# sclipman/gfa2network

Hardware: AMD Instinct MI355X
Metric: M edges/sec GFA->CSR (device-resident), + GB/s ingested (higher is better)
Workload: dtype u8/int64 (float64 weights); 1 GPU; C4: 50M S / 200M L, default (directed, MAX-SYM CSR), HBM-resident parse; n_segments=50000000, n_links=200000000, input_bytes_per_gpu=6299989066, n_nodes=50000000, nnz=289480899, mode=default, output=csr, parallelism=replica x1

## Files before the change

gfa2network_amd/_native.py:

```python
from __future__ import annotations

import ctypes
import os
import sys
from dataclasses import dataclass, field
from pathlib import Path

import numpy as np

LIB_PATH = Path(__file__).resolve().parent / "_lib" / "libg2n.so"

ABI_VERSION = 2
MAX_PHASES = 40

OK = 0
E_MALFORMED_L, E_MALFORMED_E, E_MALFORMED_C, E_MALFORMED_P, E_MALFORMED_O = 1, 2, 3, 4, 5
E_INDEX_LIST, E_INDEX_BYTES, E_UNICODE, E_INT_TOO_LARGE = 6, 7, 8, 9
E_CAST_OVERFLOW, E_CAST_INF, E_CAST_NAN = 10, 11, 12
E_ARG, E_IO, E_GZIP, E_DEVICE, E_NOMEM, E_UNSUPPORTED = 13, 14, 15, 16, 17, 18

DTYPE_CODES = {"bool": 0, "int8": 1, "int32": 2, "float32": 3, "float64": 4}
CODE_DTYPES = {v: np.dtype(k) for k, v in DTYPE_CODES.items()}
OUT_PARSE, OUT_CSR, OUT_COO, OUT_EDGE_LIST = 0, 1, 2, 3
FMT_COO, FMT_CSR, FMT_TEXT = 0, 1, 2

EXPORTED = [
    "g2n_version", "g2n_abi_version", "g2n_options_init", "g2n_device_count", "g2n_device_memory", "g2n_last_error",
    "g2n_status_name", "g2n_release_shared", "g2n_build_from_path", "g2n_build_from_buffer", "g2n_result_free",
    "g2n_coo_to_csr", "g2n_coo_to_csr_band", "g2n_context_create", "g2n_context_destroy", "g2n_context_stream", "g2n_context_trim",
    "g2n_build_device", "g2n_build_decimal_range", "g2n_count_device", "g2n_order_keys", "g2n_rank_keys", "g2n_upload_file_range", "g2n_partition_keys", "g2n_dedup_keys", "g2n_gather_keys", "g2n_remap_pairs", "g2n_route_triplets", "g2n_csr_from_coo_pair",
    "g2n_context_group_slots", "g2n_route_group_slots", "g2n_csr_from_group_slots",
    "g2n_keyset_create", "g2n_keyset_add", "g2n_keyset_view", "g2n_keyset_free",
    "g2n_gunzip", "g2n_gunzip_chunked", "g2n_free", "g2n_split_render", "g2n_split_get", "g2n_split_segments", "g2n_split_free", "g2n_join_names", "g2n_gather_names", "g2n_write_npz", "g2n_write_node_map", "g2n_first_bad_utf8",
    "g2n_csr_stats", "g2n_csr_stats_host", "g2n_stats_from_path",
]


TEST_NO_BUCKETS = 2
TEST_NO_LEAN = 4
TEST_DICT_HASH = 8
TEST_DICT_GENERAL = 16
TEST_NO_TILE_LOCAL = 32
TEST_HOST_INFLATE = 64
TEST_NO_GROUP = 128
TEST_NO_HASH_LEAN = 256
TEST_THROW_AFTER_IDS = 512
TEST_INDEX64 = 1024
TEST_DICT_DIRECT = 2048
TEST_NO_DIRECT = 4096
TEST_NO_EXT_LEAN = 8192
TEST_NO_DEC_TEXT = 16384
TEST_NO_DEC_PREFIX = 32768
TEST_FLAGS = int(os.environ.get("G2N_TEST_FLAGS", "0"), 0)
RANGE_DECIMAL = 1
RANGE_EVIDENCE = 2
RANGE_NO_VALUES = 4
RANGE_SLOTS = 8


class Options(ctypes.Structure):
    _fields_ = [
        ("abi_version", ctypes.c_uint32),
        ("directed", ctypes.c_int32),
        ("bidirected", ctypes.c_int32),
        ("keep_directed_bidir", ctypes.c_int32),
        ("asymmetric", ctypes.c_int32),
        ("strip_orientation", ctypes.c_int32),
        ("dtype", ctypes.c_int32),
        ("output", ctypes.c_int32),
        ("weight_tag", ctypes.c_char_p),
        ("want_node_names", ctypes.c_int32),
        ("device", ctypes.c_int32),
        ("unknown_warned", ctypes.c_int32),
        ("range_flags", ctypes.c_int32),
        ("range_s_base", ctypes.c_int64),
        ("range_n_segments", ctypes.c_int64),
        ("test_flags", ctypes.c_uint32),
        ("reserved_", ctypes.c_int32 * 3),
    ]


class Result(ctypes.Structure):
    _fields_ = [
        ("abi_version", ctypes.c_uint32),
        ("status", ctypes.c_int32),
# ... 697 lines not shown
```

gfa2network_amd/csrc/g2n_pipeline.hip:

```cpp
#include <hip/hip_runtime.h>

#include <chrono>
#include <cstring>
#include <functional>
#include <map>
#include <memory>
#include <mutex>

#include "g2n_internal.h"
#include "g2n_kernels.hip"
#include "g2n_scan.hip"
#include "g2n_sort.hip"
#include "g2n_sym.hip"
#include "g2n_route.hip"
#include "g2n_inflate.hip"
#include "g2n_keyset.hip"
#include "g2n_stats.hip"

#define G2N_HIP(call)                                                                                      \
  do {                                                                                                     \
    hipError_t e_ = (call);                                                                                \
    if (e_ != hipSuccess)                                                                                  \
      throw ::g2n::Failure(G2N_E_DEVICE, std::string(#call " failed: ") + hipGetErrorString(e_));          \
  } while (0)

namespace g2n {

enum Slot {
  S_IN, S_TILE_CNT, S_TILE_BASE, S_LS, S_KIND, S_NOFF, S_NLEN, S_OOFF, S_OLEN, S_EW, S_ETB, S_WL, S_TABLE,
  S_SLOT, S_FIRST, S_NID, S_FLEN, S_BLOB, S_OFFS, S_ROWS, S_COLS, S_DATA, S_KEYS0, S_KEYS1, S_VALS0, S_VALS1,
  S_KV, S_ODATA, S_INDPTR, S_INDICES, S_TEMP, S_WT, S_TKIND, S_TSTATE, S_RSTART0, S_RSTART1, S_ROUT0,
  S_ROUT1, S_UCNT0, S_UCNT1, S_UOFF, S_MCNT, S_MOFF, S_RSCR, S_RFLAG0, S_RFLAG1, S_RVAL0, S_RVAL1, S_TID,
  S_INV, S_TUNK, S_DEFER, S_FOFF64, S_BTC, S_BTV, S_BTOT, S_EBAD, S_ELEN, S_EPOS, S_ETEXT, S_EFIRST, S_EMETA, S_EL0, S_EL1,
  S_PCNT, S_POFF, S_PGRP, S_BSTART, S_SCANST, S_RBOUND, S_ROWSP, S_COLSP, S_TLEAN, S_ZIN, S_ZMEM, S_ZBAD, S_RSK, S_RSV, S_RSCNT, S_RSOFF,
  S_GCNT, S_TCN, S_INDPTR64, S_INDICES64, S_WENC, S_W1, S_W2, S_TVAL, S_PW0, S_PW1, S_BSTARTA, S_DIRECT, S_RTOT, S_SCANST2, S_EWP, S_TLIST, S_TNB, S_WENCP,
  S_STPARENT, S_STCOL, S_STDIAG, S_STLONG, S_STOUT, S_STIP, S_STIX,
  S_NSLOTS
};

constexpr uint64_t kMinGroups = 1024;
constexpr uint32_t kPtileSmallDiv = 4;
constexpr uint32_t kF2Ranges = 4;
constexpr uint32_t kTestNoBuckets = G2N_TEST_NO_BUCKETS;
constexpr uint32_t kTestNoLean = G2N_TEST_NO_LEAN;
constexpr uint32_t kTestDictHash = G2N_TEST_DICT_HASH;
constexpr uint32_t kTestDictGeneral = G2N_TEST_DICT_GENERAL;
constexpr uint32_t kTestNoTileLocal = G2N_TEST_NO_TILE_LOCAL;
constexpr uint32_t kTestNoGroup = G2N_TEST_NO_GROUP;
constexpr uint32_t kTestNoHashLean = G2N_TEST_NO_HASH_LEAN;
constexpr uint32_t kTestThrowAfterIds = G2N_TEST_THROW_AFTER_IDS;
constexpr uint32_t kTestIndex64 = G2N_TEST_INDEX64;
constexpr uint32_t kTestDictDirect = G2N_TEST_DICT_DIRECT;
constexpr uint32_t kTestNoDirect = G2N_TEST_NO_DIRECT;
constexpr uint32_t kTestNoExtLean = G2N_TEST_NO_EXT_LEAN;
constexpr uint32_t kTestNoDecText = G2N_TEST_NO_DEC_TEXT;
constexpr uint32_t kTestNoDecPrefix = G2N_TEST_NO_DEC_PREFIX;


struct DevBuf {
  void* p = nullptr;
  size_t cap = 0;
  uint64_t call = 0;
};
struct ScanSlot {
  void* p = nullptr;
  size_t cap = 0;
  uint32_t epoch = 0;
  uint64_t ticket = 0;
};

struct GroupedCoo {
  bool active = false;
  bool failed = false;
  const int32_t* rows = nullptr;
  const int32_t* cols = nullptr;
  const uint32_t* gcount = nullptr;
  uint64_t gcap = 0, n_groups = 0;
  const uint32_t* wenc = nullptr;
};

}

struct g2n_context {
  int device = 0;
  int n_cu = 256;
  uint32_t test_flags = 0;
  uint64_t err_line_off = 0;
  g2n::GroupedCoo gcoo;
  g2n::GroupedCoo slots;
// ... 334 lines not shown
  const bool words = !t_rows && (sum || !pair);
  const uint32_t ptile = n_el >= (1ull << 24) ? kPartTile : kPartTile / kPtileSmallDiv;
  src.tile = ptile;
  const uint64_t n_blk1 = grouped ? c->gcoo.n_groups : (n_el + ptile - 1) / ptile;
  const uint64_t nm1 = (uint64_t)n_dig1 * n_blk1;
  auto* cnt1 = dget<uint32_t>(c, S_PCNT, (words ? 2 : 1) * nm1);
  auto* off1 = dget<uint32_t>(c, S_POFF, (words ? 2 : 1) * nm1);
  auto* el1 = dget<uint2>(c, S_EL0, n_el);
  uint32_t* wa1 = words ? dget<uint32_t>(c, S_PW0, n_trip) : nullptr;
  if (sum && !t_rows) {
    src.pair_bits = (uint32_t)low + 1u;
    hipLaunchKernelGGL(k_part_hist<4>, dim3((unsigned)n_blk1), dim3(kPartTPB), 0, c->stream, src, shift1, n_dig1,
                       cnt1, n_blk1);
    scan_excl<uint32_t, uint32_t>(c, cnt1, off1, 2 * nm1);
    hipLaunchKernelGGL(k_part_scatter<4>, dim3((unsigned)n_blk1), dim3(kPartTPB), 0, c->stream, src, shift1, n_dig1,
                       (const uint32_t*)off1, n_blk1, el1, wa1);
  } else if (sum || pair) {
    hipLaunchKernelGGL(k_part_hist<3>, dim3((unsigned)n_blk1), dim3(kPartTPB), 0, c->stream, src, shift1, n_dig1,
                       cnt1, n_blk1);
    scan_excl<uint32_t, uint32_t>(c, cnt1, off1, (uint64_t)n_dig1 * n_blk1);
    hipLaunchKernelGGL(k_part_scatter<3>, dim3((unsigned)n_blk1), dim3(kPartTPB), 0, c->stream, src, shift1, n_dig1,
                       (const uint32_t*)off1, n_blk1, el1);
  } else {
    hipLaunchKernelGGL(k_part_hist<1>, dim3((unsigned)n_blk1), dim3(kPartTPB), 0, c->stream, src, shift1, n_dig1,
                       cnt1, n_blk1);
    scan_excl<uint32_t, uint32_t>(c, cnt1, off1, 2 * nm1);
    hipLaunchKernelGGL(k_part_scatter<1>, dim3((unsigned)n_blk1), dim3(kPartTPB), 0, c->stream, src, shift1, n_dig1,
                       (const uint32_t*)off1, n_blk1, el1, wa1);
  }
  auto* bst = dget<uint32_t>(c, S_BSTART, n_buckets + 1);
  uint32_t* bstA = words ? dget<uint32_t>(c, S_BSTARTA, n_buckets + 1) : nullptr;
  const uint2* el = el1;
  const uint32_t* wa = wa1;
  if (bits2 == 0) {
    hipLaunchKernelGGL(k_part_bucket_starts1, dim3(grid_for(n_buckets + 1)), dim3(kTPB), 0, c->stream,
                       (const uint32_t*)off1, (const uint32_t*)cnt1, n_blk1, n_buckets, bst, (const uint32_t*)nullptr);
    if (words)
      hipLaunchKernelGGL(k_part_bucket_starts1, dim3(grid_for(n_buckets + 1)), dim3(kTPB), 0, c->stream,
                         (const uint32_t*)(off1 + nm1), (const uint32_t*)(cnt1 + nm1), n_blk1, n_buckets, bstA,
                         (const uint32_t*)(off1 + nm1));
  } else {
    auto* grp = dget<uint32_t>(c, S_PGRP, 4 * ((uint64_t)n_dig1 + 1));
    uint32_t* grpA = grp + 2 * ((uint64_t)n_dig1 + 1);
    PartSrc s2{nullptr, nullptr, 0, 0, nullptr, nullptr, 0, 0, el1, grp, grp + n_dig1 + 1, n_dig1, nullptr, 0, 0};
    s2.tile = ptile;
    hipLaunchKernelGGL(k_part_groups, dim3(words ? 2 : 1), dim3(1024), 0, c->stream, (const uint32_t*)off1,
                       (const uint32_t*)cnt1, n_blk1, n_dig1, grp, ptile);
    const uint64_t n_blk2 = (n_el + ptile - 1) / ptile + n_dig1;
    const uint64_t n2 = (uint64_t)n_dig2 * n_blk2;
    const uint64_t ns = words ? 2 : 1;
    auto* cnt2 = dget<uint32_t>(c, S_PCNT, ns * n2);
    auto* off2 = dget<uint32_t>(c, S_POFF, std::max<uint64_t>(ns * n2, ns * nm1));
    auto* el2 = dget<uint2>(c, S_EL1, n_el);
    PartSrc s2a{nullptr, nullptr, 0, 0, nullptr, nullptr, 0, 0, nullptr, grpA, grpA + n_dig1 + 1, n_dig1,
                nullptr, 0, (uint32_t)low + 1u, nullptr, wa1, ptile};
    s2a.obase = off2 + n2;
    uint32_t* wa2 = words ? dget<uint32_t>(c, S_PW1, n_trip) : nullptr;
    const bool wide = bits2 > (int)kMaxDigitBits;
    if (wide) {
      hipLaunchKernelGGL((k_part_hist<2, kWideDigitBits>), dim3((unsigned)n_blk2), dim3(kPartTPB), 0, c->stream, s2,
                         (uint32_t)low, n_dig2, cnt2, n_blk2);
      if (words)
        hipLaunchKernelGGL((k_part_hist<7, kWideDigitBits>), dim3((unsigned)n_blk2), dim3(kPartTPB), 0, c->stream,
                           s2a, 2u * (uint32_t)low, n_dig2, cnt2 + n2, n_blk2);
    } else {
      hipLaunchKernelGGL(k_part_hist<2>, dim3((unsigned)n_blk2), dim3(kPartTPB), 0, c->stream, s2, (uint32_t)low,
                         n_dig2, cnt2, n_blk2);
      if (words)
        hipLaunchKernelGGL(k_part_hist<7>, dim3((unsigned)n_blk2), dim3(kPartTPB), 0, c->stream, s2a,
                           2u * (uint32_t)low, n_dig2, cnt2 + n2, n_blk2);
    }
    scan_excl<uint32_t, uint32_t>(c, cnt2, off2, ns * n2);
    if (wide)
      hipLaunchKernelGGL((k_part_scatter<2, kWideDigitBits>), dim3((unsigned)n_blk2), dim3(kPartTPB), 0, c->stream, s2,
                         (uint32_t)low, n_dig2, (const uint32_t*)off2, n_blk2, el2);
    else
      hipLaunchKernelGGL(k_part_scatter<2>, dim3((unsigned)n_blk2), dim3(kPartTPB), 0, c->stream, s2, (uint32_t)low,
                         n_dig2, (const uint32_t*)off2, n_blk2, el2);
    hipLaunchKernelGGL(k_part_bucket_starts, dim3(grid_for(n_buckets + 1)), dim3(kTPB), 0, c->stream,
                       (const uint32_t*)off2, s2, n_dig2, n_buckets, bst);
// ... 1 lines not shown
    if (words) {
      if (wide)
        hipLaunchKernelGGL((k_part_scatter<7, kWideDigitBits>), dim3((unsigned)n_blk2), dim3(kPartTPB), 0,
                           c->stream, s2a, 2u * (uint32_t)low, n_dig2, (const uint32_t*)(off2 + n2), n_blk2,
                           (uint2*)nullptr, wa2);
      else
        hipLaunchKernelGGL(k_part_scatter<7>, dim3((unsigned)n_blk2), dim3(kPartTPB), 0, c->stream, s2a,
                           2u * (uint32_t)low, n_dig2, (const uint32_t*)(off2 + n2), n_blk2, (uint2*)nullptr, wa2);
      hipLaunchKernelGGL(k_part_bucket_starts, dim3(grid_for(n_buckets + 1)), dim3(kTPB), 0, c->stream,
                         (const uint32_t*)(off2 + n2), s2a, n_dig2, n_buckets, bstA);
      wa = wa2;
    }
  }
  phase(c, "sum");
  auto* indptr = dget<int32_t>(c, S_INDPTR, n_rows + 1);
  auto* indices = dget<int32_t>(c, S_INDICES, n_el);
  T* odata = dget<T>(c, S_ODATA, n_el);
  auto* btot = dget<uint32_t>(c, S_BTOT, n_bk);
  uint2* tmp = el == el1 ? dget<uint2>(c, S_EL1, n_el) : el1;
  auto* tcol = (uint32_t*)tmp;
  auto* tcn = dget<uint16_t>(c, S_TCN, 2 * n_el);
  G2N_HIP(hipMemsetAsync(&c->ctl->bucket_overflow, 0, sizeof(unsigned long long), c->stream));
#ifdef G2N_F1_STAMPS
  unsigned long long* f1st = dget<unsigned long long>(c, S_TEMP, n_bk * kF1Stamps);
  G2N_HIP(hipMemsetAsync(f1st, 0, n_bk * kF1Stamps * 8, c->stream));
  G2N_HIP(hipMemcpyToSymbolAsync(HIP_SYMBOL(g2n_f1_stamps), &f1st, sizeof(f1st), 0, hipMemcpyHostToDevice,
                                 c->stream));
#endif
  fork_side(c);
  const uint32_t n_ov = (n_el <= 0x7FFFFFFFull && !(c->test_flags & kTestIndex64) && n_bk >= 32768ull) ? kF2Ranges : 1u;
  auto rb = [&](uint32_t k) -> uint64_t { return n_bk * k / n_ov; };
  uint32_t* boff = nullptr;
  auto launch_f1 = [&](uint64_t b0, uint64_t nb) {
    auto* f1 = sum ? k_sym_finish<T, true> : k_sym_finish<T, false>;
    hipLaunchKernelGGL(f1, dim3((unsigned)nb), dim3(kFinTPB), 0, c->stream, el, (const uint32_t*)bst, (uint32_t)low,
                       n_rows, (T)1, btot, tcol, tcn, indptr, c->ctl, (uint32_t)row_base, wa, (const uint32_t*)bstA,
                       (uint32_t)b0);
  };
  auto launch_f2 = [&](hipStream_t st, auto* ind, int64_t* ip64, uint64_t b0, uint64_t nb, const uint32_t* rt,
                       uint32_t rk) {
    using I = std::remove_pointer_t<decltype(ind)>;
    hipLaunchKernelGGL((k_sym_place<T, I>), dim3((unsigned)nb), dim3(kFinTPB), 0, st, (const uint32_t*)bst,
                       (const uint32_t*)btot, (const uint32_t*)boff, (uint32_t)low, n_rows, (T)1, (const uint32_t*)tcol,
                       (const uint16_t*)tcn, indptr, ind, odata, ip64, (const uint32_t*)bstA, (uint32_t)b0, rt, rk);
  };
  if (n_ov > 1) {
    boff = dget<uint32_t>(c, S_MOFF, n_bk + 1);
    auto* rtot = dget<uint32_t>(c, S_RTOT, n_ov);
    (void)dget<unsigned long long>(c, S_SCANST2, scan_tiles(n_bk) + 1);
    for (uint32_t k = 0; k < n_ov; k++) {
      launch_f1(rb(k), rb(k + 1) - rb(k));
      G2N_HIP(hipEventRecord(c->ov_ev[k], c->stream));
    }
    for (uint32_t k = 0; k < n_ov; k++) {
      const uint64_t b0 = rb(k), b1 = rb(k + 1);
      G2N_HIP(hipStreamWaitEvent(c->place, c->ov_ev[k], 0));
      scan_excl<uint32_t, uint32_t>(c, (const uint32_t*)(btot + b0), boff + b0, b1 - b0, rtot + k, c->place, S_SCANST2);
      launch_f2(c->place, indices, nullptr, b0, b1 - b0, rtot, k);
    }
    G2N_HIP(hipEventRecord(c->ov_ev[16], c->place));
    G2N_HIP(hipStreamWaitEvent(c->stream, c->ov_ev[16], 0));
    int32_t nnz = 0;
    G2N_HIP(hipMemcpyAsync(&nnz, indptr + n_rows, sizeof(int32_t), hipMemcpyDeviceToHost, c->stream));
    sync_ctl(c);
    if (c->h_ctl->bucket_overflow) return false;
    R->format = G2N_FMT_CSR;
    R->indptr = indptr;
    R->nnz = (int64_t)nnz;
    R->indices = indices;
    R->data = odata;
// ... 76 lines not shown
  PartSrc src{(const uint32_t*)rows, (const uint32_t*)cols, n_trip, 1u, nullptr, nullptr, 0, 0, nullptr, nullptr,
              nullptr, 0, nullptr, 0, (uint32_t)low + 1u, enc, nullptr};
  const uint32_t ptile = n_el >= (1ull << 24) ? kPartTile : kPartTile / kPtileSmallDiv;
  src.tile = ptile;
  const bool grouped = c->gcoo.active;
  if (grouped) {
    src.rows = (const uint32_t*)c->gcoo.rows;
    src.cols = (const uint32_t*)c->gcoo.cols;
    src.n_entries = c->gcoo.n_groups * c->gcoo.gcap;
    src.gcount = c->gcoo.gcount;
    src.gcap = c->gcoo.gcap;
  }
  const uint64_t n_blk1 = grouped ? c->gcoo.n_groups : (n_el + ptile - 1) / ptile;
  auto* cnt1 = dget<uint32_t>(c, S_PCNT, (uint64_t)n_dig1 * n_blk1);
  auto* off1 = dget<uint32_t>(c, S_POFF, (uint64_t)n_dig1 * n_blk1);
  auto* el1 = dget<uint2>(c, S_EL0, n_el);
  auto* w1 = dget<uint32_t>(c, S_W1, n_el);
  hipLaunchKernelGGL(k_part_hist<5>, dim3((unsigned)n_blk1), dim3(kPartTPB), 0, c->stream, src, shift1, n_dig1, cnt1,
                     n_blk1);
  scan_excl<uint32_t, uint32_t>(c, cnt1, off1, (uint64_t)n_dig1 * n_blk1);
  hipLaunchKernelGGL(k_part_scatter<5>, dim3((unsigned)n_blk1), dim3(kPartTPB), 0, c->stream, src, shift1, n_dig1,
                     (const uint32_t*)off1, n_blk1, el1, w1);
  auto* bst = dget<uint32_t>(c, S_BSTART, n_buckets + 1);
  const uint2* el = el1;
  const uint32_t* ew = w1;
  if (bits2 == 0) {
    hipLaunchKernelGGL(k_part_bucket_starts1, dim3(grid_for(n_buckets + 1)), dim3(kTPB), 0, c->stream,
                       (const uint32_t*)off1, (const uint32_t*)cnt1, n_blk1, n_buckets, bst, (const uint32_t*)nullptr);
  } else {
    auto* grp = dget<uint32_t>(c, S_PGRP, 2 * ((uint64_t)n_dig1 + 1));
    PartSrc s2{nullptr, nullptr, 0, 0, nullptr, nullptr, 0, 0, el1, grp, grp + n_dig1 + 1, n_dig1, nullptr, 0, 0,
               nullptr, w1, ptile};
    hipLaunchKernelGGL(k_part_groups, dim3(1), dim3(1024), 0, c->stream, (const uint32_t*)off1, (const uint32_t*)cnt1,
                       n_blk1, n_dig1, grp, ptile);
    const uint64_t n_blk2 = (n_el + ptile - 1) / ptile + n_dig1;
    auto* cnt2 = dget<uint32_t>(c, S_PCNT, (uint64_t)n_dig2 * n_blk2);
    auto* off2 = dget<uint32_t>(c, S_POFF, std::max<uint64_t>((uint64_t)n_dig2 * n_blk2, (uint64_t)n_dig1 * n_blk1));
    auto* el2 = dget<uint2>(c, S_EL1, n_el);
    auto* w2 = dget<uint32_t>(c, S_W2, n_el);
    hipLaunchKernelGGL(k_part_hist<6>, dim3((unsigned)n_blk2), dim3(kPartTPB), 0, c->stream, s2, (uint32_t)low,
                       n_dig2, cnt2, n_blk2);
    scan_excl<uint32_t, uint32_t>(c, cnt2, off2, (uint64_t)n_dig2 * n_blk2);
    hipLaunchKernelGGL(k_part_scatter<6>, dim3((unsigned)n_blk2), dim3(kPartTPB), 0, c->stream, s2, (uint32_t)low,
                       n_dig2, (const uint32_t*)off2, n_blk2, el2, w2);
    hipLaunchKernelGGL(k_part_bucket_starts, dim3(grid_for(n_buckets + 1)), dim3(kTPB), 0, c->stream,
                       (const uint32_t*)off2, s2, n_dig2, n_buckets, bst);
    el = el2;
    ew = w2;
  }
  phase(c, "sum");
  auto* indptr = dget<int32_t>(c, S_INDPTR, n_rows + 1);
  auto* btot = dget<uint32_t>(c, S_BTOT, n_bk);
  auto* tcol = (uint32_t*)(el == el1 ? dget<uint2>(c, S_EL1, n_el) : el1);
  T* tval = dget<T>(c, S_TVAL, 2 * n_el);
  fork_side(c);
#ifdef G2N_F1_STAMPS
  unsigned long long* f1st = dget<unsigned long long>(c, S_TEMP, n_bk * kF1Stamps);
  G2N_HIP(hipMemsetAsync(f1st, 0, n_bk * kF1Stamps * 8, c->stream));
  G2N_HIP(hipMemcpyToSymbolAsync(HIP_SYMBOL(g2n_f1_stamps), &f1st, sizeof(f1st), 0, hipMemcpyHostToDevice,
                                 c->stream));
#endif
  hipLaunchKernelGGL((k_sumw_finish<T>), dim3((unsigned)n_bk), dim3(kFinTPB), 0, c->stream, el, ew,
                     (const uint32_t*)bst, (uint32_t)low, n_rows, btot, tcol, tval, indptr, c->ctl);
#ifdef G2N_F1_STAMPS
  stamps_to_file(c, "G2N_F1_STAMPS_OUT", f1st, n_bk * kF1Stamps);
#endif
  auto* boff = dget<uint32_t>(c, S_MOFF, n_bk + 1);
// ... 2371 lines not shown
```

gfa2network_amd/csrc/g2n_sym.hip:

```cpp
#pragma once
#include <hip/hip_runtime.h>
#include <stdint.h>

#include <type_traits>

#include "g2n_kernels.h"
#include "g2n_scan.hip"

namespace g2n {

constexpr uint32_t kPartTPB = 1024;
constexpr uint32_t kSubPer = 8;
constexpr uint32_t kSub = kSubPer * kPartTPB;
constexpr uint32_t kChunkSubs = 8 * 1024 / kPartTPB;
constexpr uint32_t kPartTile = kSub * kChunkSubs;
constexpr uint32_t kMaxDigitBits = 10;
constexpr uint32_t kWideDigitBits = 11;
constexpr uint32_t kFinTPB = 256;
constexpr uint32_t kSymCap = 16 * kFinTPB;
constexpr uint32_t kSymPer = kSymCap / kFinTPB;
constexpr uint32_t kSymReg = 8;

template <uint32_t kN>
__device__ inline uint32_t block_excl_scan_n(uint32_t v, uint32_t* excl, uint32_t* lds ) {
// ... 305 lines not shown
      const uint2 y = stage[i];
      uint32_t d = (y.x >> shift) & dmask;
      if constexpr (kSplit<kPass>) {
        if ((y.y & 3u) == kElPair) {
          d += n_dig;
          wout[cur[d] + (i - hist[d])] = pair_word(y, shift, low, S.row_base);
          continue;
        }
      }
      if constexpr (kWords<kPass>) {
        wout[cur[d] + (i - hist[d])] = y.x;
      } else {
        out[cur[d] + (i - hist[d])] = y;
        if constexpr (kHasW<kPass>) wout[cur[d] + (i - hist[d])] = wstage[i];
      }
    }
    __syncthreads();
#pragma unroll
    for (uint32_t q = 0; q < kDigPer; q++) {
      const uint32_t d = threadIdx.x * kDigPer + q;
      if (d < nd) cur[d] += hv[q];
    }
    raw = nraw;
  }
}

__device__ inline uint32_t part_total(const uint32_t* offs, const uint32_t* counts, uint64_t n) {
  return n ? offs[n - 1] + counts[n - 1] : 0u;
}

__global__ void __launch_bounds__(1024) k_part_groups(const uint32_t* __restrict__ offs_all,
                                                      const uint32_t* __restrict__ cnt_all, uint64_t n_blk1,
                                                      uint32_t n_groups, uint32_t* __restrict__ gstart_all,
                                                      uint32_t tile) {
  __shared__ uint32_t red[16];
  const uint64_t nm = (uint64_t)n_groups * n_blk1;
  const uint32_t* offs1 = offs_all + blockIdx.x * nm;
  const uint32_t* cnt1 = cnt_all + blockIdx.x * nm;
  uint32_t* gstart = gstart_all + 2 * (uint64_t)blockIdx.x * (n_groups + 1);
  uint32_t* bstart = gstart + n_groups + 1;
  const uint32_t sub = blockIdx.x ? offs1[0] : 0u;
  const uint32_t g = threadIdx.x;
  const uint32_t total = part_total(offs1, cnt1, nm) - sub;
  const uint32_t s = g < n_groups ? offs1[(uint64_t)g * n_blk1] - sub : total;
  const uint32_t e = g + 1 < n_groups ? offs1[(uint64_t)(g + 1) * n_blk1] - sub : total;
  const uint32_t nb = g < n_groups ? (e - s + tile - 1) / tile : 0u;
  const int lane = threadIdx.x & 63, wid = threadIdx.x >> 6;
  uint32_t x = nb;
  for (int o = 1; o < 64; o <<= 1) {
    const uint32_t y = __shfl_up(x, o, 64);
    if (lane >= o) x += y;
  }
  if (lane == 63) red[wid] = x;
  __syncthreads();
  uint32_t base = 0, all = 0;
  for (int q = 0; q < 16; q++) {
    if (q < wid) base += red[q];
    all += red[q];
  }
  if (g < n_groups) {
    gstart[g] = s;
    bstart[g] = base + x - nb;
  }
  if (g == 0) {
    gstart[n_groups] = total;
    bstart[n_groups] = all;
  }
}

__global__ void __launch_bounds__(kTPB) k_part_bucket_starts(const uint32_t* __restrict__ offs2, PartSrc m,
                                                             uint32_t n_dig2, uint64_t n_buckets,
                                                             uint32_t* __restrict__ bstart_out) {
  const uint64_t q = (uint64_t)blockIdx.x * kTPB + threadIdx.x;
  if (q > n_buckets) return;
  if (q == n_buckets) {
    bstart_out[q] = m.gstart[m.n_groups];
    return;
  }
  const uint32_t g = (uint32_t)(q / n_dig2), d = (uint32_t)(q % n_dig2);
  const uint32_t nb = m.bstart[g + 1] - m.bstart[g];
  bstart_out[q] = nb ? offs2[(uint64_t)m.bstart[g] * n_dig2 + (uint64_t)d * nb] - (m.obase ? *m.obase : 0u)
                     : m.gstart[g];
}

__global__ void __launch_bounds__(kTPB) k_part_bucket_starts1(const uint32_t* __restrict__ offs1,
                                                              const uint32_t* __restrict__ cnt1, uint64_t n_blk1,
                                                              uint64_t n_buckets, uint32_t* __restrict__ bstart_out,
                                                              const uint32_t* __restrict__ sub) {
  const uint64_t q = (uint64_t)blockIdx.x * kTPB + threadIdx.x;
  if (q > n_buckets) return;
  bstart_out[q] = (q == n_buckets ? part_total(offs1, cnt1, n_buckets * n_blk1) : offs1[q * n_blk1]) - (sub ? *sub : 0u);
}

__device__ inline void sym_sort_row(uint32_t* seg, uint32_t n) {
  if (n <= 1) return;
  if (n <= 16) {
    uint32_t k[16];
#pragma unroll
    for (uint32_t q = 0; q < 16; q++) k[q] = q < n ? seg[q] : 0xFFFFFFFFu;
    if (n <= 4) net_sort<4>(k);
    else if (n <= 8) net_sort<8>(k);
    else net_sort<16>(k);
#pragma unroll
    for (uint32_t q = 0; q < 16; q++)
      if (q < n) seg[q] = k[q];
    return;
  }
  constexpr uint32_t gaps[8] = {701, 301, 132, 57, 23, 10, 4, 1};
  for (uint32_t gp : gaps) {
    if (gp >= n) continue;
    for (uint32_t i = gp; i < n; i++) {
      const uint32_t v = seg[i];
      uint32_t jj = i;
      while (jj >= gp && seg[jj - gp] > v) {
        seg[jj] = seg[jj - gp];
        jj -= gp;
      }
      seg[jj] = v;
    }
  }
}

constexpr uint32_t kShortRow = 16;
constexpr uint32_t kMidRow = 64;
// ... 17 lines not shown
template <class Keep, class Emit>
__device__ inline uint32_t wave_merge(uint32_t x, uint32_t nr, Keep keep, Emit emit) {
  const uint32_t lane = threadIdx.x & 63;
  const uint32_t col = x >> 1, sd = x & 1u;
  const bool valid = lane < nr;
  const uint32_t pcol = (uint32_t)__shfl_up((int)col, 1, 64), ncol = (uint32_t)__shfl_down((int)col, 1, 64);
  const bool start = valid && (lane == 0 || pcol != col);
  const bool last = valid && (lane + 1 == nr || ncol != col);
  const unsigned long long smask = __ballot(start), s1 = __ballot(valid && sd);
  const unsigned long long upto = (2ull << lane) - 1ull;
  const uint32_t sl = 63u - (uint32_t)__clzll((smask & upto) | 1ull);
  const unsigned long long run = upto & ~((1ull << sl) - 1ull);
  const uint32_t ky = (uint32_t)__popcll(s1 & run), kx = lane - sl + 1 - ky;
  uint32_t kk = 0;
  const bool kept = last && keep(kx, ky, kk);
  const unsigned long long km = __ballot(kept);
  if (kept) emit((uint32_t)__popcll(km & ((1ull << lane) - 1ull)), col, kk);
  return (uint32_t)__popcll(km);
}

#ifdef G2N_F1_STAMPS
constexpr int kF1Stamps = 10;
__device__ unsigned long long* g2n_f1_stamps;
#define F1_STAMP(k)                                                                          \
  do {                                                                                       \
    if (threadIdx.x == 0) g2n_f1_stamps[blockIdx.x * kF1Stamps + (k)] = wall_clock64();      \
  } while (0)
#else
#define F1_STAMP(k) \
  do {              \
  } while (0)
#endif

template <class T, bool kSum>
__global__ void __launch_bounds__(kFinTPB) __attribute__((amdgpu_waves_per_eu(8, 8))) k_sym_finish(const uint2* __restrict__ el, const uint32_t* __restrict__ bstart,
                                                     uint32_t low, uint64_t n_rows, T one, uint32_t* __restrict__ btot,
                                                     uint32_t* __restrict__ tcol, uint16_t* __restrict__ tcn,
                                                     int32_t* __restrict__ indptr, Ctl* ctl, uint32_t row_base, const uint32_t* __restrict__ wa,
                                                     const uint32_t* __restrict__ bstA, uint32_t b0) {
  __shared__ __attribute__((aligned(16))) uint32_t seg[kSymCap];
  __shared__ uint32_t cnt[kFinTPB];
  __shared__ uint32_t cur[kFinTPB];
  __shared__ uint32_t red[kFinTPB / 64];
  __shared__ uint16_t mlist[kFinTPB];
  __shared__ uint32_t mval[kFinTPB];
  __shared__ uint32_t mcount;
  F1_STAMP(0);
  cnt[threadIdx.x] = 0;
  if (threadIdx.x == 0) mcount = 0;
  const uint64_t b = b0 + blockIdx.x;
  const uint32_t eB = bstart[b], nB = bstart[b + 1] - eB;
  const uint32_t eA = bstA ? bstA[b] : 0u, nA = bstA ? bstA[b + 1] - eA : 0u;
  const uint32_t e0 = eB + eA, n = nB + nA;
  auto overflow = [&]() {
    if (threadIdx.x == 0) {
      ctl->bucket_overflow = 1;
      btot[b] = 0;
    }
  };
  if (n > kSymCap) {
    overflow();
    return;
  }
  __syncthreads();
  const uint32_t rmask = (1u << low) - 1u;
  uint32_t my, rs, nx;
  {
    const uint32_t hi = (uint32_t)b << low;
    auto word = [&](uint32_t w) {
      return make_uint2(hi | ((w >> low) & rmask), (((hi | (w & rmask)) + row_base) << 2) | kElPair);
    };
    const uint32_t nr = bstA ? nA : nB;
    uint2 xs[kSymReg];
    uint2 xb = make_uint2(0, 0);
    if (bstA) {
      uint32_t ws[kSymReg];
#pragma unroll
      for (uint32_t k = 0; k < kSymReg; k++) {
        const uint32_t i = threadIdx.x + k * kFinTPB;
        ws[k] = i < nr ? wa[eA + i] : 0u;
      }
      if (threadIdx.x < nB) xb = el[eB + threadIdx.x];
#pragma unroll
      for (uint32_t k = 0; k < kSymReg; k++) xs[k] = word(ws[k]);
    } else {
#pragma unroll
      for (uint32_t k = 0; k < kSymReg; k++) {
        const uint32_t i = threadIdx.x + k * kFinTPB;
        if (i < nr) xs[k] = el[eB + i];
      }
    }
    auto count = [&](uint2 x) {
      atomicAdd(&cnt[x.x & rmask], 1u);
      if ((x.y & 3u) == kElPair) atomicAdd(&cnt[((x.y >> 2) - row_base) & rmask], 1u);
    };
    auto place = [&](uint2 x) {
      const uint32_t kind = x.y & 3u, col = x.y >> 2;
      seg[atomicAdd(&cur[x.x & rmask], 1u)] = (col << 1) | (kind & 1u);
      if (kind == kElPair)
        seg[atomicAdd(&cur[(col - row_base) & rmask], 1u)] = ((x.x + row_base) << 1) | (kSum ? 0u : 1u);
    };
#pragma unroll
    for (uint32_t k = 0; k < kSymReg; k++)
      if (threadIdx.x + k * kFinTPB < nr) count(xs[k]);
    for (uint32_t i = threadIdx.x + kSymReg * kFinTPB; i < nr; i += kFinTPB) count(bstA ? word(wa[eA + i]) : el[eB + i]);
    if (bstA) {
      if (threadIdx.x < nB) count(xb);
      for (uint32_t i = threadIdx.x + kFinTPB; i < nB; i += kFinTPB) count(el[eB + i]);
    }
    __syncthreads();
    F1_STAMP(1);
    my = cnt[threadIdx.x];
    nx = block_excl_scan_n<kFinTPB>(my, &rs, red);
    if (nx > kSymCap) {
      overflow();
      return;
    }
    cnt[threadIdx.x] = rs;
    cur[threadIdx.x] = rs;
    __syncthreads();
#pragma unroll
    for (uint32_t k = 0; k < kSymReg; k++)
      if (threadIdx.x + k * kFinTPB < nr) place(xs[k]);
    for (uint32_t i = threadIdx.x + kSymReg * kFinTPB; i < nr; i += kFinTPB) place(bstA ? word(wa[eA + i]) : el[eB + i]);
    if (bstA) {
      if (threadIdx.x < nB) place(xb);
      for (uint32_t i = threadIdx.x + kFinTPB; i < nB; i += kFinTPB) place(el[eB + i]);
    }
    __syncthreads();
    F1_STAMP(2);
  }
  const uint64_t row = (b << low) + threadIdx.x;
  const bool live = threadIdx.x <= rmask && row < n_rows;
  const bool shortrow = my <= kShortRow;
  const bool midrow = live && !shortrow && my <= kMidRow;
  const bool longrow = live && my > kMidRow;
  uint32_t* sg = seg + rs;
  const uint32_t lane = threadIdx.x & 63, wv = threadIdx.x >> 6;
  if (midrow) mlist[atomicAdd(&mcount, 1u)] = (uint16_t)threadIdx.x;
  __syncthreads();
  const uint32_t n_mid = mcount;
  uint32_t k[kShortRow];
#pragma unroll
  for (uint32_t q = 0; q < kShortRow; q++) k[q] = (live && shortrow && q < my) ? sg[q] : 0xFFFFFFFFu;
  {
    uint32_t wm = (live && shortrow) ? my : 0u;
    for (int o = 32; o > 0; o >>= 1) wm = max(wm, (uint32_t)__shfl_xor(wm, o, 64));
    if (wm > 8) net_sort<16>(k);
    else if (wm > 4) net_sort<8>(k);
    else if (wm > 1) net_sort<4>(k);
  }
  if (longrow) sym_sort_row(sg, my);
  auto keep = [&](uint32_t kx, uint32_t ky, uint32_t& kk) -> bool {
    if constexpr (kSum) {
      kk = kx;
      return true;
    } else if constexpr (std::is_same<T, int8_t>::value) {
      const T x = kx ? sum_copies<T>(one, kx) : (T)0, y = ky ? sum_copies<T>(one, ky) : (T)0;
      kk = (x < y) ? ky : kx;
      return ((x < y) ? y : x) != (T)0;
    } else {
      kk = kx > ky ? kx : ky;
      return kk != 0;
// ... 477 lines not shown
```

include/g2n.h:

```cpp
#ifndef G2N_H
#define G2N_H

#include <stddef.h>
#include <stdint.h>

#define G2N_VERSION_STRING "0.3.0"

#ifdef __cplusplus
extern "C" {
#endif

#define G2N_ABI_VERSION 2u

enum {
  G2N_OK = 0,
  G2N_E_MALFORMED_L = 1,
  G2N_E_MALFORMED_E = 2,
  G2N_E_MALFORMED_C = 3,
  G2N_E_MALFORMED_P = 4,
  G2N_E_MALFORMED_O = 5,
  G2N_E_INDEX_LIST = 6,
  G2N_E_INDEX_BYTES = 7,
  G2N_E_UNICODE = 8,
  G2N_E_INT_TOO_LARGE = 9,
// ... 25 lines not shown
  const char *weight_tag;
  int32_t want_node_names;
  int32_t device;
  int32_t unknown_warned;
  int32_t range_flags;
  int64_t range_s_base;
  int64_t range_n_segments;
  uint32_t test_flags;
  int32_t reserved_[3];
} g2n_options;

enum {
  G2N_RANGE_DECIMAL = 1,
  G2N_RANGE_EVIDENCE = 2,
  G2N_RANGE_NO_VALUES = 4,
  G2N_RANGE_SLOTS = 8
};

enum {
  G2N_TEST_NO_BUCKETS = 2,
  G2N_TEST_NO_LEAN = 4,
  G2N_TEST_DICT_HASH = 8,
  G2N_TEST_DICT_GENERAL = 16,
  G2N_TEST_NO_TILE_LOCAL = 32,
  G2N_TEST_HOST_INFLATE = 64,
  G2N_TEST_NO_GROUP = 128,
  G2N_TEST_NO_HASH_LEAN = 256,
  G2N_TEST_THROW_AFTER_IDS = 512,
  G2N_TEST_INDEX64 = 1024,
  G2N_TEST_DICT_DIRECT = 2048,
  G2N_TEST_NO_DIRECT = 4096,
  G2N_TEST_NO_EXT_LEAN = 8192,
  G2N_TEST_NO_DEC_TEXT = 16384,
  G2N_TEST_NO_DEC_PREFIX = 32768
};

#define G2N_MAX_PHASES 40

typedef struct g2n_result {
  uint32_t abi_version;
  int32_t status;
  int64_t err_line;
  int64_t err_index;
  double err_value;
  const uint8_t *err_detail;
  int64_t err_detail_len;
  int32_t has_warning;
  int32_t warn_byte;
  int64_t warn_line;
  int64_t n_lines;
  int64_t n_records;
  int64_t n_records_before_error;
  int64_t n_edges;
  int64_t n_nodes;
  const uint8_t *names_blob;
  const int64_t *names_offsets;
  int32_t format;
  int32_t dtype;
  int32_t index_width;
  int32_t sum_sorted;
  int64_t nnz;
  const void *rows;
  const void *cols;
  const void *indptr;
  const void *indices;
  const void *data;
  uint64_t names_bytes;
// ... 138 lines not shown
```

Baseline: 27650 M edge records/s.

## Replace global pass-2 partition scatter with block-local sort and run-walking finish

The second radix partition pass now sorts each chunk in place within the block (registers plus LDS staging) and records per-chunk digit offsets, instead of doing a global histogram, scan and scatter into a second buffer. Bucket starts come from summing the per-chunk run lengths, and the symmetric-finish kernel reads each bucket by walking those runs across chunks. This removes a full scatter pass and its global scan over the edge array. The cost is non-contiguous gathers and extra run-table scans inside the finish kernel, plus heavy register pressure in the local-sort kernel.

```diff
diff --git a/gfa2network_amd/_native.py b/gfa2network_amd/_native.py
--- a/gfa2network_amd/_native.py
+++ b/gfa2network_amd/_native.py
@@ -51,6 +51,8 @@
 TEST_NO_EXT_LEAN = 8192
 TEST_NO_DEC_TEXT = 16384
 TEST_NO_DEC_PREFIX = 32768
+TEST_CLASSIC_PASS2 = 65536
+TEST_SMALL_CHUNK = 131072
 TEST_FLAGS = int(os.environ.get("G2N_TEST_FLAGS", "0"), 0)
 RANGE_DECIMAL = 1
 RANGE_EVIDENCE = 2
diff --git a/gfa2network_amd/csrc/g2n_pipeline.hip b/gfa2network_amd/csrc/g2n_pipeline.hip
--- a/gfa2network_amd/csrc/g2n_pipeline.hip
+++ b/gfa2network_amd/csrc/g2n_pipeline.hip
@@ -34,6 +34,7 @@
   S_INV, S_TUNK, S_DEFER, S_FOFF64, S_BTC, S_BTV, S_BTOT, S_EBAD, S_ELEN, S_EPOS, S_ETEXT, S_EFIRST, S_EMETA, S_EL0, S_EL1,
   S_PCNT, S_POFF, S_PGRP, S_BSTART, S_SCANST, S_RBOUND, S_ROWSP, S_COLSP, S_TLEAN, S_ZIN, S_ZMEM, S_ZBAD, S_RSK, S_RSV, S_RSCNT, S_RSOFF,
   S_GCNT, S_TCN, S_INDPTR64, S_INDICES64, S_WENC, S_W1, S_W2, S_TVAL, S_PW0, S_PW1, S_BSTARTA, S_DIRECT, S_RTOT, S_SCANST2, S_EWP, S_TLIST, S_TNB, S_WENCP,
+  S_PROWS, S_BCNT,
   S_STPARENT, S_STCOL, S_STDIAG, S_STLONG, S_STOUT, S_STIP, S_STIX,
   S_NSLOTS
 };
@@ -55,6 +56,8 @@
 constexpr uint32_t kTestNoExtLean = G2N_TEST_NO_EXT_LEAN;
 constexpr uint32_t kTestNoDecText = G2N_TEST_NO_DEC_TEXT;
 constexpr uint32_t kTestNoDecPrefix = G2N_TEST_NO_DEC_PREFIX;
+constexpr uint32_t kTestClassicPass2 = G2N_TEST_CLASSIC_PASS2;
+constexpr uint32_t kTestSmallChunk = G2N_TEST_SMALL_CHUNK;
 
 
 struct DevBuf {
@@ -455,7 +458,41 @@
   uint32_t* bstA = words ? dget<uint32_t>(c, S_BSTARTA, n_buckets + 1) : nullptr;
   const uint2* el = el1;
   const uint32_t* wa = wa1;
-  if (bits2 == 0) {
+  PartRuns runs;
+  if (bits2 > 0 && bits2 <= (int)kMaxDigitBits && !(c->test_flags & kTestClassicPass2)) {
+    const bool small = (c->test_flags & kTestSmallChunk) != 0;
+    const uint32_t tile_a = small ? 64u : ptile;
+    const uint32_t tile_b = tile_a / 2;
+    auto* grp = dget<uint32_t>(c, S_PGRP, 4 * ((uint64_t)n_dig1 + 1));
+    uint32_t* grpA = grp + 2 * ((uint64_t)n_dig1 + 1);
+    hipLaunchKernelGGL(k_part_groups, dim3(words ? 2 : 1), dim3(1024), 0, c->stream, (const uint32_t*)off1,
+                       (const uint32_t*)cnt1, n_blk1, n_dig1, grp, tile_b, tile_a);
+    const uint64_t n_blk2 = (n_el + tile_b - 1) / tile_b + n_dig1;
+    const uint64_t n_blk2a = words ? (n_trip + tile_a - 1) / tile_a + n_dig1 : 0;
+    auto* prow = dget<uint32_t>(c, S_PROWS, (n_blk2 + n_blk2a) * ((uint64_t)n_dig2 + 1));
+    PartSrc s2{nullptr, nullptr, 0, 0, nullptr, nullptr, 0, 0, el1, grp, grp + n_dig1 + 1, n_dig1, nullptr, 0, 0};
+    s2.tile = tile_b;
+    PartSrc s2a{nullptr, nullptr, 0, 0, nullptr, nullptr, 0, 0, nullptr, grpA, grpA + n_dig1 + 1, n_dig1,
+                nullptr, 0, (uint32_t)low + 1u, nullptr, wa1, tile_a};
+    runs.rows = prow;
+    runs.rows_a = prow + n_blk2 * ((uint64_t)n_dig2 + 1);
+    runs.grp = grp;
+    runs.grp_a = grpA;
+    runs.n_groups = n_dig1;
+    runs.bits2 = (uint32_t)bits2;
+    runs.tile = tile_b;
+    runs.tile_a = tile_a;
+    hipLaunchKernelGGL(k_part_local<2>, dim3((unsigned)n_blk2), dim3(kPartTPB), 0, c->stream, s2, (uint32_t)low, n_dig2,
+                       el1, (uint32_t*)nullptr, prow);
+    if (words)
+      hipLaunchKernelGGL(k_part_local<7>, dim3((unsigned)n_blk2a), dim3(kPartTPB), 0, c->stream, s2a,
+                         2u * (uint32_t)low, n_dig2, (uint2*)nullptr, wa1, prow + n_blk2 * ((uint64_t)n_dig2 + 1));
+    auto* bcnt = dget<uint32_t>(c, S_BCNT, 2 * (n_buckets + 1));
+    hipLaunchKernelGGL(k_part_run_totals, dim3(grid_for(n_buckets + 1), words ? 2 : 1), dim3(kTPB), 0, c->stream, runs,
+                       n_buckets, bcnt, bcnt + n_buckets + 1);
+    scan_excl<uint32_t, uint32_t>(c, (const uint32_t*)bcnt, bst, n_buckets + 1);
+    if (words) scan_excl<uint32_t, uint32_t>(c, (const uint32_t*)(bcnt + n_buckets + 1), bstA, n_buckets + 1);
+  } else if (bits2 == 0) {
     hipLaunchKernelGGL(k_part_bucket_starts1, dim3(grid_for(n_buckets + 1)), dim3(kTPB), 0, c->stream,
                        (const uint32_t*)off1, (const uint32_t*)cnt1, n_blk1, n_buckets, bst, (const uint32_t*)nullptr);
     if (words)
@@ -468,7 +505,7 @@
     PartSrc s2{nullptr, nullptr, 0, 0, nullptr, nullptr, 0, 0, el1, grp, grp + n_dig1 + 1, n_dig1, nullptr, 0, 0};
     s2.tile = ptile;
     hipLaunchKernelGGL(k_part_groups, dim3(words ? 2 : 1), dim3(1024), 0, c->stream, (const uint32_t*)off1,
-                       (const uint32_t*)cnt1, n_blk1, n_dig1, grp, ptile);
+                       (const uint32_t*)cnt1, n_blk1, n_dig1, grp, ptile, ptile);
     const uint64_t n_blk2 = (n_el + ptile - 1) / ptile + n_dig1;
     const uint64_t n2 = (uint64_t)n_dig2 * n_blk2;
     const uint64_t ns = words ? 2 : 1;
@@ -536,10 +573,11 @@
   auto rb = [&](uint32_t k) -> uint64_t { return n_bk * k / n_ov; };
   uint32_t* boff = nullptr;
   auto launch_f1 = [&](uint64_t b0, uint64_t nb) {
-    auto* f1 = sum ? k_sym_finish<T, true> : k_sym_finish<T, false>;
+    auto* f1 = runs.rows ? (sum ? k_sym_finish<T, true, true> : k_sym_finish<T, false, true>)
+                         : (sum ? k_sym_finish<T, true, false> : k_sym_finish<T, false, false>);
     hipLaunchKernelGGL(f1, dim3((unsigned)nb), dim3(kFinTPB), 0, c->stream, el, (const uint32_t*)bst, (uint32_t)low,
                        n_rows, (T)1, btot, tcol, tcn, indptr, c->ctl, (uint32_t)row_base, wa, (const uint32_t*)bstA,
-                       (uint32_t)b0);
+                       (uint32_t)b0, runs);
   };
   auto launch_f2 = [&](hipStream_t st, auto* ind, int64_t* ip64, uint64_t b0, uint64_t nb, const uint32_t* rt,
                        uint32_t rk) {
@@ -682,7 +720,7 @@
     PartSrc s2{nullptr, nullptr, 0, 0, nullptr, nullptr, 0, 0, el1, grp, grp + n_dig1 + 1, n_dig1, nullptr, 0, 0,
                nullptr, w1, ptile};
     hipLaunchKernelGGL(k_part_groups, dim3(1), dim3(1024), 0, c->stream, (const uint32_t*)off1, (const uint32_t*)cnt1,
-                       n_blk1, n_dig1, grp, ptile);
+                       n_blk1, n_dig1, grp, ptile, ptile);
     const uint64_t n_blk2 = (n_el + ptile - 1) / ptile + n_dig1;
     auto* cnt2 = dget<uint32_t>(c, S_PCNT, (uint64_t)n_dig2 * n_blk2);
     auto* off2 = dget<uint32_t>(c, S_POFF, std::max<uint64_t>((uint64_t)n_dig2 * n_blk2, (uint64_t)n_dig1 * n_blk1));
diff --git a/gfa2network_amd/csrc/g2n_sym.hip b/gfa2network_amd/csrc/g2n_sym.hip
--- a/gfa2network_amd/csrc/g2n_sym.hip
+++ b/gfa2network_amd/csrc/g2n_sym.hip
@@ -361,8 +361,9 @@
 __global__ void __launch_bounds__(1024) k_part_groups(const uint32_t* __restrict__ offs_all,
                                                       const uint32_t* __restrict__ cnt_all, uint64_t n_blk1,
                                                       uint32_t n_groups, uint32_t* __restrict__ gstart_all,
-                                                      uint32_t tile) {
+                                                      uint32_t tile_b, uint32_t tile_a) {
   __shared__ uint32_t red[16];
+  const uint32_t tile = blockIdx.x ? tile_a : tile_b;
   const uint64_t nm = (uint64_t)n_groups * n_blk1;
   const uint32_t* offs1 = offs_all + blockIdx.x * nm;
   const uint32_t* cnt1 = cnt_all + blockIdx.x * nm;
@@ -419,6 +420,131 @@
   const uint64_t q = (uint64_t)blockIdx.x * kTPB + threadIdx.x;
   if (q > n_buckets) return;
   bstart_out[q] = (q == n_buckets ? part_total(offs1, cnt1, n_buckets * n_blk1) : offs1[q * n_blk1]) - (sub ? *sub : 0u);
+}
+
+constexpr uint32_t kLocSlots = 64;
+constexpr uint32_t kLocTile = kLocSlots * kPartTPB;
+constexpr uint32_t kLocStage = 32768;
+static_assert(kPartTile <= kLocTile, "a pass-2 chunk must fit the block's registers");
+
+template <int kPass>
+__global__ void __launch_bounds__(kPartTPB) __attribute__((amdgpu_waves_per_eu(4)))
+    k_part_local(PartSrc S, uint32_t shift, uint32_t n_dig, uint2* __restrict__ el, uint32_t* __restrict__ wa,
+                 uint32_t* __restrict__ rows) {
+  constexpr bool kW = kWords<kPass>;
+  using E = std::conditional_t<kW, uint32_t, uint2>;
+  constexpr uint32_t kN = kLocSlots * 4 / sizeof(E);
+  constexpr uint32_t kCap = kLocStage * 4 / sizeof(E);
+  __shared__ uint32_t hist[1u << kMaxDigitBits];
+  __shared__ E stage[kCap];
+  __shared__ uint32_t red[kPartTPB / 64];
+  PartBlock B;
+  if (!part_block<kPass>(S, blockIdx.x, B)) return;
+  const uint32_t n = (uint32_t)(B.e1 - B.e0);
+  E* io;
+  if constexpr (kW) io = wa + B.e0;
+  else io = el + B.e0;
+  const uint32_t dmask = n_dig - 1;
+  auto digit = [&](const E& v) -> uint32_t {
+    if constexpr (kW) return (v >> shift) & dmask;
+    else return (v.x >> shift) & dmask;
+  };
+  const uint32_t per = ((n + kPartTPB / 64 - 1) / (kPartTPB / 64) + 63u) & ~63u;
+  const uint32_t lane = threadIdx.x & 63, w0 = (threadIdx.x >> 6) * per;
+  const E* in = io + w0 + lane;
+  const uint32_t lim = n > w0 ? (n - w0 < per ? n - w0 : per) : 0u;
+  uint32_t nk = lane < lim ? (lim - lane + 63u) / 64u : 0u;
+  auto held = [&](uint32_t k) -> bool { return k < nk; };
+  hist[threadIdx.x] = 0;
+  E v[kN];
+#pragma unroll
+  for (uint32_t k = 0; k < kN; k++)
+    if (held(k)) v[k] = in[k * 64];
+  auto fresh = [&]() {
+    asm volatile("" : "+v"(nk));
+#pragma unroll
+    for (uint32_t k = 0; k < kN; k++) {
+      if constexpr (kW) asm volatile("" : "+v"(v[k]));
+      else asm volatile("" : "+v"(v[k].x));
+    }
+  };
+  __syncthreads();
+  fresh();
+  uint32_t rk[kW ? 1 : kN / 2];
+#pragma unroll
+  for (uint32_t k = 0; k < kN; k++) {
+    if constexpr (kW) {
+      if (held(k)) atomicAdd(&hist[digit(v[k])], 1u);
+    } else {
+      const uint32_t r = held(k) ? atomicAdd(&hist[digit(v[k])], 1u) : 0u;
+      rk[k / 2] = (k & 1) ? (rk[k / 2] | (r << 16)) : r;
+    }
+    if (k % 16 == 15) __builtin_amdgcn_sched_barrier(0);
+  }
+  __syncthreads();
+  const uint32_t h = hist[threadIdx.x];
+  uint32_t ex;
+  block_excl_scan_n<kPartTPB>(h, &ex, red);
+  hist[threadIdx.x] = ex;
+  uint32_t* row = rows + (uint64_t)blockIdx.x * (n_dig + 1);
+  if (threadIdx.x < n_dig) row[threadIdx.x] = ex;
+  if (threadIdx.x == 0) row[n_dig] = n;
+  __syncthreads();
+  fresh();
+  if constexpr (kW) {
+#pragma unroll
+    for (uint32_t k = 0; k < kN; k++) {
+      if (held(k)) v[k] = (atomicAdd(&hist[digit(v[k])], 1u) << 16) | (v[k] & ((1u << shift) - 1u));
+      if (k % 16 == 15) __builtin_amdgcn_sched_barrier(0);
+    }
+  }
+  for (uint32_t h0 = 0; h0 < n; h0 += kCap) {
+    fresh();
+#pragma unroll
+    for (uint32_t k = 0; k < kN; k++) {
+      if (held(k)) {
+        if constexpr (kW) {
+          const uint32_t at = (v[k] >> 16) - h0;
+          if (at < kCap) stage[at] = v[k] & 0xFFFFu;
+        } else {
+          const uint32_t at = hist[digit(v[k])] + ((rk[k / 2] >> (16 * (k & 1))) & 0xFFFFu) - h0;
+          if (at < kCap) stage[at] = v[k];
+        }
+      }
+      if (k % 16 == 15) __builtin_amdgcn_sched_barrier(0);
+    }
+    __syncthreads();
+    const uint32_t m = n - h0 < kCap ? n - h0 : kCap;
+    for (uint32_t i = threadIdx.x; i < m; i += kPartTPB) io[h0 + i] = stage[i];
+    __syncthreads();
+  }
+}
+
+struct PartRuns {
+  const uint32_t* rows = nullptr;
+  const uint32_t* rows_a = nullptr;
+  const uint32_t* grp = nullptr;
+  const uint32_t* grp_a = nullptr;
+  uint32_t n_groups = 0, bits2 = 0;
+  uint32_t tile = 0, tile_a = 0;
+};
+
+__global__ void __launch_bounds__(kTPB) k_part_run_totals(PartRuns R, uint64_t n_buckets, uint32_t* __restrict__ cnt_b,
+                                                          uint32_t* __restrict__ cnt_a) {
+  const uint64_t q = (uint64_t)blockIdx.x * kTPB + threadIdx.x;
+  if (q > n_buckets) return;
+  uint32_t* cnt = blockIdx.y ? cnt_a : cnt_b;
+  if (q == n_buckets) {
+    cnt[q] = 0;
+    return;
+  }
+  const uint32_t* rows = blockIdx.y ? R.rows_a : R.rows;
+  const uint32_t* first = (blockIdx.y ? R.grp_a : R.grp) + R.n_groups + 1;
+  const uint32_t g = (uint32_t)(q >> R.bits2), d = (uint32_t)q & ((1u << R.bits2) - 1u);
+  const uint64_t stride = (1u << R.bits2) + 1u;
+  uint32_t s = 0;
+  for (uint32_t j = first[g]; j < first[g + 1]; j++) s += rows[j * stride + d + 1] - rows[j * stride + d];
+  cnt[q] = s;
 }
 
 __device__ inline void sym_sort_row(uint32_t* seg, uint32_t n) {
@@ -502,12 +628,12 @@
   } while (0)
 #endif
 
-template <class T, bool kSum>
+template <class T, bool kSum, bool kRuns = false>
 __global__ void __launch_bounds__(kFinTPB) __attribute__((amdgpu_waves_per_eu(8, 8))) k_sym_finish(const uint2* __restrict__ el, const uint32_t* __restrict__ bstart,
                                                      uint32_t low, uint64_t n_rows, T one, uint32_t* __restrict__ btot,
                                                      uint32_t* __restrict__ tcol, uint16_t* __restrict__ tcn,
                                                      int32_t* __restrict__ indptr, Ctl* ctl, uint32_t row_base, const uint32_t* __restrict__ wa,
-                                                     const uint32_t* __restrict__ bstA, uint32_t b0) {
+                                                     const uint32_t* __restrict__ bstA, uint32_t b0, PartRuns R) {
   __shared__ __attribute__((aligned(16))) uint32_t seg[kSymCap];
   __shared__ uint32_t cnt[kFinTPB];
   __shared__ uint32_t cur[kFinTPB];
@@ -540,26 +666,6 @@
     auto word = [&](uint32_t w) {
       return make_uint2(hi | ((w >> low) & rmask), (((hi | (w & rmask)) + row_base) << 2) | kElPair);
     };
-    const uint32_t nr = bstA ? nA : nB;
-    uint2 xs[kSymReg];
-    uint2 xb = make_uint2(0, 0);
-    if (bstA) {
-      uint32_t ws[kSymReg];
-#pragma unroll
-      for (uint32_t k = 0; k < kSymReg; k++) {
-        const uint32_t i = threadIdx.x + k * kFinTPB;
-        ws[k] = i < nr ? wa[eA + i] : 0u;
-      }
-      if (threadIdx.x < nB) xb = el[eB + threadIdx.x];
-#pragma unroll
-      for (uint32_t k = 0; k < kSymReg; k++) xs[k] = word(ws[k]);
-    } else {
-#pragma unroll
-      for (uint32_t k = 0; k < kSymReg; k++) {
-        const uint32_t i = threadIdx.x + k * kFinTPB;
-        if (i < nr) xs[k] = el[eB + i];
-      }
-    }
     auto count = [&](uint2 x) {
       atomicAdd(&cnt[x.x & rmask], 1u);
       if ((x.y & 3u) == kElPair) atomicAdd(&cnt[((x.y >> 2) - row_base) & rmask], 1u);
@@ -570,6 +676,127 @@
       if (kind == kElPair)
         seg[atomicAdd(&cur[(col - row_base) & rmask], 1u)] = ((x.x + row_base) << 1) | (kSum ? 0u : 1u);
     };
+    if constexpr (kRuns) {
+      uint32_t* rst = mval;
+      uint16_t* rend = mlist;
+      const uint32_t d = (uint32_t)b & ((1u << R.bits2) - 1u), g = (uint32_t)(b >> R.bits2);
+      const uint32_t stride = (1u << R.bits2) + 1u;
+      const uint32_t* firstB = R.grp + R.n_groups + 1;
+      const uint32_t gB = R.grp[g], fB = firstB[g], nbB = firstB[g + 1] - fB;
+      uint32_t gA = 0, fA = 0, nbA = 0;
+      if (bstA) {
+        const uint32_t* firstA = R.grp_a + R.n_groups + 1;
+        gA = R.grp_a[g];
+        fA = firstA[g];
+        nbA = firstA[g + 1] - fA;
+      }
+      const uint32_t n_runs = nbA + nbB;
+      uint32_t totA, tot;
+      auto build = [&](uint32_t q0) {
+        const uint32_t q = q0 + threadIdx.x;
+        uint32_t len = 0, st = 0;
+        if (q < n_runs) {
+          const bool a = q < nbA;
+          const uint32_t j = a ? q : q - nbA;
+          const uint32_t* row = (a ? R.rows_a + (uint64_t)(fA + j) * stride : R.rows + (uint64_t)(fB + j) * stride) + d;
+          const uint32_t o0 = row[0];
+          len = row[1] - o0;
+          st = (a ? gA + j * R.tile_a : gB + j * R.tile) + o0;
+        }
+        uint32_t ex;
+        tot = block_excl_scan_n<kFinTPB>(len, &ex, red);
+        rst[threadIdx.x] = st - ex;
+        rend[threadIdx.x] = (uint16_t)(ex + len);
+        __syncthreads();
+        const uint32_t na = nbA > q0 ? (nbA - q0 < kFinTPB ? nbA - q0 : kFinTPB) : 0u;
+        totA = na ? rend[na - 1] : 0u;
+      };
+      auto walk = [&](uint32_t i, uint32_t& r) -> uint32_t {
+        while (i >= rend[r]) r++;
+        return rst[r] + i;
+      };
+      auto rest = [&](uint32_t a0, uint32_t b0, auto fn) {
+        uint32_t r = 0;
+        for (uint32_t i = threadIdx.x + a0 * kFinTPB; i < totA; i += kFinTPB) fn(word(wa[walk(i, r)]));
+        for (uint32_t i = totA + threadIdx.x + b0 * kFinTPB; i < tot; i += kFinTPB) fn(el[walk(i, r)]);
+      };
+      build(0);
+      const uint32_t a0 = bstA ? kSymReg : 0u, b0 = bstA ? 1u : kSymReg;
+      const uint32_t rA = totA, rT = tot;
+      uint2 xs[kSymReg];
+      uint2 xb = make_uint2(0, 0);
+      if (bstA) {
+        uint32_t ws[kSymReg], r = 0;
+#pragma unroll
+        for (uint32_t k = 0; k < kSymReg; k++) {
+          const uint32_t i = threadIdx.x + k * kFinTPB;
+          ws[k] = i < rA ? wa[walk(i, r)] : 0u;
+        }
+        if (rA + threadIdx.x < rT) xb = el[walk(rA + threadIdx.x, r)];
+#pragma unroll
+        for (uint32_t k = 0; k < kSymReg; k++) xs[k] = word(ws[k]);
+      } else {
+        uint32_t r = 0;
+#pragma unroll
+        for (uint32_t k = 0; k < kSymReg; k++) {
+          const uint32_t i = threadIdx.x + k * kFinTPB;
+          if (i < rT) xs[k] = el[walk(i, r)];
+        }
+      }
+      const uint32_t nr = bstA ? rA : rT;
+      auto regs = [&](auto fn) {
+#pragma unroll
+        for (uint32_t k = 0; k < kSymReg; k++)
+          if (threadIdx.x + k * kFinTPB < nr) fn(xs[k]);
+        if (bstA && rA + threadIdx.x < rT) fn(xb);
+      };
+      regs(count);
+      rest(a0, b0, count);
+      for (uint32_t q0 = kFinTPB; q0 < n_runs; q0 += kFinTPB) {
+        build(q0);
+        rest(0u, 0u, count);
+      }
+      __syncthreads();
+      F1_STAMP(1);
+      my = cnt[threadIdx.x];
+      nx = block_excl_scan_n<kFinTPB>(my, &rs, red);
+      if (nx > kSymCap) {
+        overflow();
+        return;
+      }
+      cnt[threadIdx.x] = rs;
+      cur[threadIdx.x] = rs;
+      if (n_runs > kFinTPB) build(0);
+      else __syncthreads();
+      regs(place);
+      rest(a0, b0, place);
+      for (uint32_t q0 = kFinTPB; q0 < n_runs; q0 += kFinTPB) {
+        build(q0);
+        rest(0u, 0u, place);
+      }
+      __syncthreads();
+      F1_STAMP(2);
+    } else {
+    const uint32_t nr = bstA ? nA : nB;
+    uint2 xs[kSymReg];
+    uint2 xb = make_uint2(0, 0);
+    if (bstA) {
+      uint32_t ws[kSymReg];
+#pragma unroll
+      for (uint32_t k = 0; k < kSymReg; k++) {
+        const uint32_t i = threadIdx.x + k * kFinTPB;
+        ws[k] = i < nr ? wa[eA + i] : 0u;
+      }
+      if (threadIdx.x < nB) xb = el[eB + threadIdx.x];
+#pragma unroll
+      for (uint32_t k = 0; k < kSymReg; k++) xs[k] = word(ws[k]);
+    } else {
+#pragma unroll
+      for (uint32_t k = 0; k < kSymReg; k++) {
+        const uint32_t i = threadIdx.x + k * kFinTPB;
+        if (i < nr) xs[k] = el[eB + i];
+      }
+    }
 #pragma unroll
     for (uint32_t k = 0; k < kSymReg; k++)
       if (threadIdx.x + k * kFinTPB < nr) count(xs[k]);
@@ -599,6 +826,7 @@
     }
     __syncthreads();
     F1_STAMP(2);
+    }
   }
   const uint64_t row = (b << low) + threadIdx.x;
   const bool live = threadIdx.x <= rmask && row < n_rows;
diff --git a/include/g2n.h b/include/g2n.h
--- a/include/g2n.h
+++ b/include/g2n.h
@@ -81,7 +81,9 @@
   G2N_TEST_NO_DIRECT = 4096,
   G2N_TEST_NO_EXT_LEAN = 8192,
   G2N_TEST_NO_DEC_TEXT = 16384,
-  G2N_TEST_NO_DEC_PREFIX = 32768
+  G2N_TEST_NO_DEC_PREFIX = 32768,
+  G2N_TEST_CLASSIC_PASS2 = 65536,
+  G2N_TEST_SMALL_CHUNK = 131072
 };
 
 #define G2N_MAX_PHASES 40
```

Result: slower. 27130 M edge records/s (-1.9%).
